# ruihuang1124/CAFE-MPC

Hardware: AMD Instinct MI355X
Metric: DDP iterations/sec, Mini-Cheetah WB N=200, batch=4096; 1/2/4/8 GPU (higher is better)
Workload: dtype f64

## Files before the change

### cafe-mpc_amd/csrc/wb_knot.hpp

```cpp
#pragma once
#include "hs_types.hpp"
#include "wb_model.hpp"
#include "hs_mfma.hpp"

namespace hs {

struct WbCore {
    double x[36], xb[36], u[12], acc[18], tau[18], fext[12], cs[18], sn[18];
    double M[18 * 18];
    double h[18], Jall[12 * 18], Jdv[12], fpos[12], fvel[12];
    double JX[432];
    double gam[12];
    double GG[288 + 2 * MAXG];
    HD double* Jc() { return JX; }
    HD double* Xm() { return JX + 216; }
    HD double* G() { return GG; }
    HD double* LG() { return GG + 144; }
    HD double* gval() { return GG + 288; }
    HD double* bar() { return GG + 288 + MAXG; }
    HD double* dacc() { return GG; }
    HD double* dvel() { return GG + 216; }
    double a0[18], rhs[12], lam[12], qdd[18], grf[12], tmp[64], red[64], rdM[18], rdG[12];
    double wq[48];
    double xnext[36];
// ... 160 lines not shown
        wb_pass<double>(c, L.x, L.x + 18, L.acc, L.cs, L.sn, L.fext, sk);
        if (tid < 12) {
            for (int f = 0; f < 4; f++) if (f != leg) {
                for (int r = 0; r < 3; r++) { L.M[(3 * f + r) * 18 + wb_pj(col)] = 0.0; L.Jall[(3 * f + r) * 18 + col] = 0.0; }
            }
        }
    })
    HS_PHASE(NT, if (tid < 19 && (need_cols || tid == 18)) {
        const int t0 = (tid < 6) ? 12 + 4 * tid : (tid < 18) ? tid - 6 : 36, nt = (tid < 6 || tid == 18) ? 4 : 1;
        V3<double> fb = {0.0, 0.0, 0.0}, nb = fb;
        for (int t = 0; t < nt; t++) { const double* p = L.GG + 6 * (t0 + t); fb = fb + V3<double>{p[0], p[1], p[2]}; nb = nb + V3<double>{p[3], p[4], p[5]}; }
        PSink sk{&L, tid, 0};
        const double c3 = L.cs[3], s3 = L.sn[3], c4 = L.cs[4], s4 = L.sn[4], c5 = L.cs[5], s5 = L.sn[5];
        sk.tau(5, nb.x);
        V3<double> f = rot<0, double>(c5, s5, fb), n = rot<0, double>(c5, s5, nb);
        sk.tau(4, n.y);
        f = rot<1, double>(c4, s4, f); n = rot<1, double>(c4, s4, n);
        sk.tau(3, n.z);
        f = rot<2, double>(c3, s3, f);
        sk.tau(0, f.x); sk.tau(1, f.y); sk.tau(2, f.z);
    })
}

struct Feet4 { int f0, f1, f2, f3; HD int operator[](int i) const { return i == 0 ? f0 : i == 1 ? f1 : i == 2 ? f2 : f3; }
    HD int pick(int i) const { return (((f0 & 3) | (f1 & 3) << 2 | (f2 & 3) << 4 | (f3 & 3) << 6) >> (2 * i)) & 3; } };
HD Feet4 feet_of(PhaseC& P) { int f0 = P.feet[0], f1 = P.feet[1], f2 = P.feet[2], f3 = P.feet[3]; HS_PIN_S(f0); HS_PIN_S(f1); HS_PIN_S(f2); HS_PIN_S(f3); return Feet4{f0, f1, f2, f3}; }
template <class T> HD double pick3(const T& w, int a) { const double w0 = w[0], w1 = w[1], w2 = w[2]; return a == 0 ? w0 : a == 1 ? w1 : w2; }

template <int NT>
HD void wb_select(WbCore& L, int nc, const Feet4& feet, int mode, double alpha) {
    HS_PHASE(NT,
        for (int e = tid; e < 216; e += NT) {
            const int a = e / 18, j = e % 18; const bool act = a < 3 * nc;
            L.Jc()[e] = act ? L.Jall[(3 * feet.pick(act ? a / 3 : 0) + a % 3) * 18 + wb_pi(j)] : 0.0;
        }
        for (int e = tid; e < 144; e += NT) L.G()[e] = (e % 13 == 0) ? 1.0 : 0.0;
        if (tid < 12) {
            const bool act = tid < 3 * nc;
            const int f = act ? feet.pick(tid / 3) : 0, r = tid % 3;
            L.gam[tid] = (act && mode == 0) ? (L.Jdv[3 * f + r] + 2.0 * alpha * L.fvel[3 * f + r]) : 0.0;
            L.grf[tid] = 0.0;
        })
}
template <int NM> HD void wb_gram(WbCore& L, int m, int tid, int nt) {
    for (int e = tid; e < NM * NM; e += nt) {
        const int a = e / NM, b = e % NM;
        double s = 0;
        _Pragma("unroll")
        for (int i = 0; i < 18; i++) s += L.Xm()[i * 12 + a] * L.Xm()[i * 12 + b];
        if (a < m && b < m) L.G()[a * 12 + b] = s;
    }
}

template <int NT, int NM>
HD void wb_kkt_tail(WbCore& L, int m, const Feet4& feet, int mode) {
    HS_PHASE(NT, wb_gram<NM>(L, m, tid, NT);
        if (tid >= 48 && tid < 60) {
            const int a = tid - 48; double s = 0;
            if (mode == 0) { _Pragma("unroll") for (int i = 0; i < 18; i++) s += L.Xm()[i * 12 + a] * L.a0[i]; }
            else { _Pragma("unroll") for (int i = 0; i < 18; i++) s += L.Jc()[a * 18 + i] * L.x[18 + wb_pi(i)]; }
            L.rhs[a] = (a < m) ? (-s - L.gam[a]) : 0.0;
        })
    LQ_STAMP(9)
    chol_f<NT, NM, 12>(L.G(), L.LG(), L.rdG, (mode == 0) ? 1e-12 : 0.0);
    LQ_STAMP(10)
#ifdef HS_HOST_EMU
    HS_PHASE(NT, if (tid == 0) {
        double lam[12];
        _Pragma("unroll")
        for (int i = 0; i < 12; i++) lam[i] = L.rhs[i];
        fwd_s<NM, 12>(L.LG(), L.rdG, lam); bwd_s<NM, 12>(L.LG(), L.rdG, lam);
        double z[18];
        _Pragma("unroll")
        for (int i = 0; i < 18; i++) { double s = L.a0[i]; _Pragma("unroll") for (int a = 0; a < NM; a++) s += L.Xm()[i * 12 + a] * lam[a]; z[i] = s; }
        bwd_s<18, 18, WbNZ>(L.M, L.rdM, z);
        _Pragma("unroll")
        for (int i = 0; i < 18; i++) L.qdd[wb_pi(i)] = z[i] + ((mode == 1) ? L.x[18 + wb_pi(i)] : 0.0);
        _Pragma("unroll")
        for (int a = 0; a < 12; a++) { L.lam[a] = lam[a]; if (a < m) L.grf[3 * feet[a / 3] + a % 3] = lam[a]; }
    })
#else
    HS_PHASE(NT, {
        const int i12 = tid < NM ? tid : NM - 1, i18 = tid < 18 ? tid : 17;
        double lgr[NM], lgc[NM], xr[NM], lmc[6], lleg[3];
        _Pragma("unroll") for (int k = 0; k < NM; k++) { lgr[k] = L.LG()[i12 * 12 + k]; lgc[k] = L.LG()[k * 12 + i12]; xr[k] = L.Xm()[i18 * 12 + k]; }
        const int lg = i18 < 12 ? i18 / 3 : 3, jl = i18 - 3 * lg;
        _Pragma("unroll") for (int k = 0; k < 6; k++) lmc[k] = L.M[(12 + k) * 18 + i18];
        _Pragma("unroll") for (int j = 0; j < 3; j++) lleg[j] = L.M[(3 * lg + j) * 18 + i18];
        const double rg = L.rdG[i12], rm = L.rdM[i18];
        double v = L.rhs[i12];
        _Pragma("unroll") for (int k = 0; k < NM; k++) { const double xk = hs_readlane(v * rg, k); v = (tid == k) ? xk : ((tid > k) ? v - lgr[k] * xk : v); }
        _Pragma("unroll") for (int k = NM - 1; k >= 0; k--) { const double xk = hs_readlane(v * rg, k); v = (tid == k) ? xk : ((tid < k) ? v - lgc[k] * xk : v); }
        double z = L.a0[i18];
        _Pragma("unroll") for (int a = 0; a < NM; a++) z += xr[a] * hs_readlane(v, a);
        _Pragma("unroll") for (int k = 17; k >= 12; k--) { const double xk = hs_readlane(z * rm, k); z = (tid == k) ? xk : ((tid < k) ? z - lmc[k - 12] * xk : z); }
        _Pragma("unroll") for (int j = 2; j >= 0; j--) { const double xk = hs_bperm(z * rm, 3 * lg + j); z = (tid < 12 && jl == j) ? xk : ((tid < 12 && jl < j) ? z - lleg[j] * xk : z); }
        if (tid < 18) L.qdd[wb_pi(tid)] = z + ((mode == 1) ? L.x[18 + wb_pi(tid)] : 0.0);
        if (tid < 12) { const double lm = tid < NM ? v : 0.0; L.lam[tid] = lm; if (tid < m) L.grf[3 * feet.pick(tid / 3) + tid % 3] = lm; }
    })
#endif
}

template <int NT>
HD void wb_kkt_direct(WbCore& L, int nc, const Feet4& feet, int mode, double alpha) {
    const int m = 3 * nc;
    wb_select<NT>(L, nc, feet, mode, alpha);
    LQ_STAMP(7)
#ifdef HS_HOST_EMU
    chol_f<NT, 18, 18, WbNZ>(L.M, L.M, L.rdM, 0.0);
#else
    HS_PHASE(NT, chol_wb18(L.M, L.rdM, tid);)
#endif
    LQ_STAMP(8)
    HS_PHASE(NT, if (tid < 13) {
        const bool isx = tid < 12;
        double* w = reinterpret_cast<double*>(&L);
        constexpr int OXM = offsetof(WbCore, JX) / 8 + 216, OA0 = offsetof(WbCore, a0) / 8;
        double x[18];
        _Pragma("unroll")
        for (int i = 0; i < 18; i++) {
            const double jc = L.Jc()[(isx ? tid : 0) * 18 + i], yv = (mode == 0) ? (L.tau[wb_pi(i)] - L.h[wb_pi(i)]) : 0.0;
            x[i] = isx ? jc : yv;
        }
        fwd_s<18, 18, WbNZ>(L.M, L.rdM, x);
        const int o0 = isx ? OXM + tid : OA0, st = isx ? 12 : 1;
        _Pragma("unroll")
        for (int i = 0; i < 18; i++) w[o0 + i * st] = x[i];
    })
    if (m <= 6) wb_kkt_tail<NT, 6>(L, m, feet, mode); else wb_kkt_tail<NT, 12>(L, m, feet, mode);
}

template <int NM> HD void wb_kkt_column_mid(const WbCore& L, const WbDeriv& D, double* top, double* bot) {
    _Pragma("unroll")
    for (int a = 0; a < NM; a++) {
        double s = -bot[a];
        _Pragma("unroll")
        for (int i = 0; i < 18; i++) s += L.JX[216 + i * 12 + a] * top[i];
        bot[a] = s;
    }
    fwd_s<NM, 12>(D.LGs, D.rdGs, bot); bwd_s<NM, 12>(D.LGs, D.rdGs, bot);
    _Pragma("unroll")
    for (int i = 0; i < 18; i++) {
        double s = top[i];
        _Pragma("unroll")
        for (int a = 0; a < NM; a++) s -= L.JX[216 + i * 12 + a] * bot[a];
        top[i] = s;
    }
}
HD void wb_kkt_column(const WbCore& L, const WbDeriv& D, double* top, double* bot, bool top_is_y, int m) {
    if (!top_is_y) fwd_s<18, 18, WbNZ>(L.M, L.rdM, top);
    if (m <= 6) wb_kkt_column_mid<6>(L, D, top, bot); else wb_kkt_column_mid<12>(L, D, top, bot);
    bwd_s<18, 18, WbNZ>(L.M, L.rdM, top);
}
template <int NT> HD void wb_keep_schur(WbCore& L, WbDeriv& D) {
    chol_f<NT, 12, 12>(L.G(), D.LGs, D.rdGs, 0.0);
}

template <int NT>
HD void wb_dpass(WbCore& L, WbDeriv& D, const ModelDev& md, double grav, double vscale_dyn, double vscale_kin, double ascale_kin, bool q_only, bool chol_g = false) {
    auto base_seed = [](int bs) { return bs < 3 ? 3 + bs : bs < 6 ? 36 + bs : 12 + bs; };
    auto zero_rest = [&](int seed, int leg) {
        for (int f = 0; f < 4; f++) if (f != leg) for (int r = 0; r < 3; r++) {
            D.W[(6 + 3 * f + r) * WT + seed] = 0.0;
            if (seed >= 36) { L.dacc()[(3 * f + r) * 18 + seed - 36] = 0.0; L.dvel()[(3 * f + r) * 18 + seed - 36] = 0.0; }
        }
    };
    HS_PHASE(NT,
        WB_W1_STAMP_BEGIN()
        if (tid < 60 && !(q_only && ((tid >= 12 && tid < 36) || tid >= 48))) {
            const int t = tid; int seed, leg, slot = 0; bool part = t < 36;
            if (t < 12) { seed = base_seed(t >> 2); leg = t & 3; slot = t; }
            else if (t < 36) { const int bs = 6 + ((t - 12) >> 2); seed = base_seed(bs); leg = t & 3; slot = 4 * bs + leg; }
            else { const int jl = (t - 36) % 12; seed = (t < 48 ? 6 : 24) + jl; leg = jl / 3; }
            LaneCfg c = lane_cfg(md, false, 1.0, grav, 0.0, vscale_dyn, 1.0, -1, seed < 18 ? seed : -1, seed >= 18 ? seed - 18 : -1);
            c.l0 = leg; c.l1 = leg + 1; c.body = part && leg == 0; c.partial = part;
            DSink sk{&D, &L, seed, slot};
            wb_pass<Dual, DSink, 1>(c, L.x, L.x + 18, L.acc, L.cs, L.sn, L.fext, sk);
            if (!part) zero_rest(seed, leg);
        }
        const int kt = (NT >= 128) ? tid - 64 : tid;
        if (kt >= 0 && kt < 24) {
            const int t = kt; int seed, leg, slot = 0; const bool part = t < 12;
            if (part) { const int bs = 3 + (t >> 2); seed = base_seed(bs); leg = t & 3; slot = 4 * bs + leg; }
            else { const int jl = t - 12; seed = 42 + jl; leg = jl / 3; }
            LaneCfg c = lane_cfg(md, true, 0.0, 0.0, 1.0, vscale_kin, ascale_kin, -1, seed - 36, -1);
            c.l0 = leg; c.l1 = leg + 1; c.body = false; c.partial = part;
            DSink sk{&D, &L, seed, slot};
            wb_pass<Dual, DSink, 2>(c, L.x, L.x + 18, L.acc, L.cs, L.sn, L.fext, sk);
            if (!part) zero_rest(seed, leg);
        }
        for (int e = tid; e < 108; e += NT) { const int sd = e / 18, i = e % 18; D.W[i * WT + (sd < 3 ? sd : 33 + sd)] = 0.0; }
        for (int e = tid; e < 36; e += NT) { const int j = e / 12, r = e % 12; L.dacc()[r * 18 + j] = 0.0; L.dvel()[r * 18 + j] = 0.0; }
        if (NT >= 128 && chol_g && tid >= 64) WB_CHOL_G(D.LGs, D.rdGs, tid - 64);
        WB_W1_STAMP_END(6))
    HS_PHASE(NT, if (tid < (q_only ? 6 : 12)) {
        const int seed = base_seed(tid), tq = seed < 18 ? seed : seed >= 36 ? seed - 36 : -1;
        V3<Dual> fb = {Dual(0.0), Dual(0.0), Dual(0.0)}, nb = fb;
        for (int l = 0; l < 4; l++) {
            const double* p = D.JPW + 12 * (4 * tid + l);
            fb = fb + V3<Dual>{Dual(p[0], p[1]), Dual(p[2], p[3]), Dual(p[4], p[5])}; nb = nb + V3<Dual>{Dual(p[6], p[7]), Dual(p[8], p[9]), Dual(p[10], p[11])};
        }
        auto SC = [&](int i, Dual& s_, Dual& c_) { const double c0 = L.cs[i], s0 = L.sn[i]; const bool sd = (tq == i); s_ = Dual(s0, sd ? c0 : 0.0); c_ = Dual(c0, sd ? -s0 : 0.0); };
        Dual c3, s3, c4, s4, c5, s5;
        SC(3, s3, c3); SC(4, s4, c4); SC(5, s5, c5);
        DSink sk{&D, &L, seed, 0};
        sk.tau(5, nb.x);
        V3<Dual> f = rot<0>(c5, s5, fb), n = rot<0>(c5, s5, nb);
        sk.tau(4, n.y);
        f = rot<1>(c4, s4, f); n = rot<1>(c4, s4, n);
        sk.tau(3, n.z);
        f = rot<2>(c3, s3, f);
        sk.tau(0, f.x); sk.tau(1, f.y); sk.tau(2, f.z);
    })
}

HD double reb_barrier(double g, double delta) {
    if (g > delta) return -log(g);
    double t = (g - 2 * delta) / delta;
    return .5 * (t * t - 1) - log(delta);
}

HD double wb_constraint(PhaseC& P, const WbCore& L, int c) {
    if (P.go_torque >= 0 && c >= P.go_torque && c < P.go_torque + 24) { int i = c - P.go_torque; return i < 12 ? -L.u[i] + P.torque_limit : L.u[i - 12] + P.torque_limit; }
    if (P.go_jspeed >= 0 && c >= P.go_jspeed && c < P.go_jspeed + 24) { int i = c - P.go_jspeed; return i < 12 ? L.x[24 + i] - P.jspeed_lb : -L.x[24 + i - 12] + P.jspeed_ub; }
    if (P.go_joint >= 0 && c >= P.go_joint && c < P.go_joint + 24) { int i = c - P.go_joint; return i < 12 ? L.x[6 + i] - pick3(P.joint_lb, i % 3) : -L.x[6 + i - 12] + pick3(P.joint_ub, i % 3); }
    if (P.go_height >= 0 && c == P.go_height) return L.x[2] - P.h_min;
    int i = c - P.go_grf, a = i / 5, r = i % 5, f = feet_of(P)[a];
    double fx = L.grf[3 * f], fy = L.grf[3 * f + 1], fz = L.grf[3 * f + 2];
    if (r == 0) return fz;
    if (r == 1) return -fx + P.mu * fz;
    if (r == 2) return fx + P.mu * fz;
    if (r == 3) return -fy + P.mu * fz;
    return fy + P.mu * fz;
}

HD double wb_constraint_sel(PhaseC& P, const WbCore& L, int c) {
    const double* w = reinterpret_cast<const double*>(&L);
    constexpr int OX = offsetof(WbCore, x) / 8, OU = offsetof(WbCore, u) / 8, OG = offsetof(WbCore, grf) / 8;
    const int it = c - P.go_torque, is = c - P.go_jspeed, ij = c - P.go_joint;
    const bool bt = P.go_torque >= 0 && it >= 0 && it < 24, bs = P.go_jspeed >= 0 && is >= 0 && is < 24, bj = P.go_joint >= 0 && ij >= 0 && ij < 24;
    const bool bh = P.go_height >= 0 && c == P.go_height, lin = bt || bs || bj || bh;
    const int i = bt ? it : bs ? is : ij, lo = i < 12 ? i : i - 12;
    const bool up = i >= 12;
    const int a3 = lo % 3;
    const double cj = up ? pick3(P.joint_ub, a3) : -pick3(P.joint_lb, a3);
    const double c0 = bt ? P.torque_limit : bs ? (up ? P.jspeed_ub : -P.jspeed_lb) : bj ? cj : -P.h_min;
    const double sg = bt ? (up ? 1.0 : -1.0) : (bh || !up) ? 1.0 : -1.0;
    const int i1l = bt ? OU + lo : bs ? OX + 24 + lo : bj ? OX + 6 + lo : OX + 2;
    const int ig = lin ? 0 : c - P.go_grf, ga = ig / 5, gr = ig - 5 * ga, f = feet_of(P).pick(ga & 3);
    const int i1 = lin ? i1l : OG + 3 * f + 2, i2 = lin ? i1l : OG + 3 * f + (gr >= 3 ? 1 : 0);
    const double v1 = w[i1], v2 = w[i2];
    const double a = lin ? sg : (gr == 0 ? 1.0 : P.mu);
    const double t2 = lin ? c0 : (gr == 0 ? 0.0 : ((gr == 1 || gr == 3) ? -v2 : v2));
    return hs_fma(a, v1, t2);
}
HD double reb_barrier1(double g, double delta) {
    const bool above = g > delta;
    const double lg = log(above ? g : delta);
    double q = 0.0;
    if (!above) { const double t = (g - 2 * delta) / delta; q = .5 * (t * t - 1); }
    return above ? -lg : q - lg;
}

struct SlotOut { double* cost; double* dsq; double* ming; double* maxh; };

template <int NT, int CNT, int ROWS, class DST, class F>
HD void store_image(DST dst, int tid, F f) {
    constexpr int R = (CNT + NT - 1) / NT;
    const int c0 = tid / ROWS, r0 = tid - ROWS * c0;
    double v[R];
    _Pragma("unroll")
    for (int q = 0; q < R; q++) {
        const int e = tid + NT * q; int r = r0 + (NT * q) % ROWS, c = c0 + (NT * q) / ROWS;
        if (r >= ROWS) { r -= ROWS; c++; }
        v[q] = 0.0;
        if (R * NT == CNT || e < CNT) v[q] = f(e, r, c);
    }
    _Pragma("unroll")
    for (int q = 0; q < R; q++) { const int e = tid + NT * q; if (R * NT == CNT || e < CNT) dst[e] = v[q]; }
}

template <int NT>
HD void wb_rollout_knot(WbCore& L, PhaseC& P, const ModelDev& md, int b, int k, double eps, int reb_active,
                        const double* x0, SlotOut so, size_t slot, int* fail_flag, bool ss = false, bool wr = true) {
    const int h = P.h;
    const size_t kx = ((size_t)b * (h + 1) + k) * 36, ku = ((size_t)b * h + k) * 12;
    double* Kst = L.Jc();
    RL_STAMP0()
    const size_t kk = (size_t)b * h + k;
    struct Late { double kr[7]; } late[HS_NLANES(NT)];
    HS_PHASE(NT,
        const int g = tid < 36 ? 0 : tid < 48 ? 1 : tid < 60 ? 2 : 3, i = tid < 36 ? tid : tid < 48 ? tid - 36 : tid < 60 ? tid - 48 : 0;
        const double* pa = g == 0 ? P.Xbar + kx + i : (g == 1 && !ss) ? P.KdX + ku + i : P.Xbar + kx; const double* pb = P.dX + kx + (g == 0 ? i : 0);
        const double* rr = P.rref + ref_row(P, b, k) * 80;
        const double* pc = rr + tid;
        const double* pd = g == 0 ? P.Xbar + kx + (ss ? 0 : 36) + i : g == 1 ? P.Ubar + ku + i : rr + 64 + i;
        const double* pe = g == 0 ? P.dX + kx + (ss ? 0 : 36) + i : g == 1 ? P.dU + ku + i : rr;
        double va = *pa, vb = *pb, vc = *pc, vd = *pd, ve = *pe;
        const double* pw = tid < 36 ? &P.q[tid] : &P.r[tid < 48 ? tid - 36 : 0];
        const double vw = *pw;
        double er[2], dr[2];
        _Pragma("unroll") for (int q = 0; q < 2; q++) { const int c = q * NT + tid; er[q] = (c < P.ng) ? P.eps[kk * P.ng + c] : 0.0; dr[q] = (c < P.ng) ? P.delta[kk * P.ng + c] : 0.0; }
        if (ss) { Late& lt = late[HS_LANE(tid)]; _Pragma("unroll") for (int q = 0; q < 7; q++) { const int e = q * NT + tid; lt.kr[q] = (e < 432) ? P.K[kk * 432 + e] : 0.0; } }
        HS_CBAR();
        if (tid < 36) {
            const double xb = va, x = ss ? L.xnext[tid] : xb + eps * vb;
// ... 203 lines not shown
    double g = 0;
    for (int f = 0; f < 4; f++) {
        const double* wp = D.wp + 3 * f; const double* wv = D.wv + 3 * f;
        const double* J0 = Jall + (3 * f) * 18; const double* J1 = J0 + 18; const double* J2 = J1 + 18;
        if (wp[0] != 0.0 || wp[1] != 0.0 || wp[2] != 0.0) {
            const bool in = d >= 3 && d < 18; const int dd = in ? d : 3;
            const double t0 = in ? wp[0] * J0[dd] : 0.0, t1 = in ? wp[1] * J1[dd] : 0.0, t2 = in ? wp[2] * J2[dd] : 0.0;
            g += t0 * D.ep[3 * f] + t1 * D.ep[3 * f + 1] + t2 * D.ep[3 * f + 2];
            _Pragma("unroll")
            for (int i = 3; i < 18; i++) acc[i] += J0[i] * t0 + J1[i] * t1 + J2[i] * t2;
        }
        if (wv[0] != 0.0 || wv[1] != 0.0 || wv[2] != 0.0) {
            const double* V0 = dvel + (3 * f) * 18; const double* V1 = V0 + 18; const double* V2 = V1 + 18;
            const int dd = d < 18 ? d : d - 18;
            const double t0 = wv[0] * (d < 18 ? V0[dd] : J0[dd]), t1 = wv[1] * (d < 18 ? V1[dd] : J1[dd]), t2 = wv[2] * (d < 18 ? V2[dd] : J2[dd]);
            g += t0 * D.ev[3 * f] + t1 * D.ev[3 * f + 1] + t2 * D.ev[3 * f + 2];
            _Pragma("unroll")
            for (int i = 0; i < 18; i++) { acc[i] += V0[i] * t0 + V1[i] * t1 + V2[i] * t2; acc[18 + i] += J0[i] * t0 + J1[i] * t1 + J2[i] * t2; }
        }
    }
    _Pragma("unroll")
    for (int i = 0; i < 36; i++) colout[i * 36] = acc[i];
    return g;
}

#ifndef HS_HOST_EMU
HD void wb_cost_gram_acc(WbCore& L, WbDeriv& D, int lane, d4_t (&c)[3][3]) {
    const int li = lane & 15, lk = lane >> 4;
    bool anyv = false;
    _Pragma("unroll") for (int a = 0; a < 12; a++) anyv = anyv || (D.wv[a] != 0.0);
    _Pragma("unroll") for (int ti = 0; ti < 3; ti++) _Pragma("unroll") for (int tj = 0; tj < 3; tj++) c[ti][tj] = d4_t{0.0, 0.0, 0.0, 0.0};
    _Pragma("unroll") for (int kg = 0; kg < 6; kg++) {
        if (kg >= 3 && !anyv) break;
        const int k = 4 * kg + lk, r = (kg < 3) ? k : k - 12;
        const double w = (kg < 3) ? D.wp[r] : D.wv[r], res = (kg < 3) ? D.ep[r] : D.ev[r];
        double e[3];
        _Pragma("unroll") for (int t = 0; t < 3; t++) {
            const int col = 16 * t + li, cc = col < 36 ? col : 35, lo = cc < 18, c18 = lo ? cc : cc - 18;
            const double vj = L.Jall[r * 18 + c18];
            if (kg < 3) e[t] = (cc >= 3 && lo && col < 36) ? vj : 0.0;
            else { const double vd = L.dvel()[r * 18 + c18]; e[t] = col < 36 ? (lo ? vd : vj) : 0.0; }
        }
        _Pragma("unroll") for (int ti = 0; ti < 3; ti++) {
            const double a = w * e[ti];
            _Pragma("unroll") for (int tj = 0; tj < 3; tj++) {
                const double bb = (tj == 2 && li == 4) ? res : e[tj];
                c[ti][tj] = __builtin_amdgcn_mfma_f64_16x16x4f64(a, bb, c[ti][tj], 0, 0, 0);
            }
        }
    }
}
#endif
template <int NT>
HD void wb_cost_gram(WbLqLds& S, double* gvec) {
    WbCore& L = S.c; WbDeriv& D = S.d;
#ifdef HS_HOST_EMU
    HS_PHASE_L(NT, if (tid < 37) {
        const int j = tid;
        auto E = [&](int k, int c) { if (k < 12) return (c >= 3 && c < 18) ? L.Jall[k * 18 + c] : 0.0; const int r = k - 12; return c < 18 ? L.dvel()[r * 18 + c] : L.Jall[r * 18 + c - 18]; };
        for (int i = 0; i < 36; i++) {
            double s = 0;
            for (int k = 0; k < 24; k++) { const double w = k < 12 ? D.wp[k] : D.wv[k - 12]; s += w * E(k, i) * (j < 36 ? E(k, j) : (k < 12 ? D.ep[k] : D.ev[k - 12])); }
            if (j < 36) D.W[i * 36 + j] = s; else gvec[i] = s;
        }
    })
#else
    HS_PHASE_L(NT, if (tid < 64) {
        const int li = tid & 15, lk = tid >> 4;
        d4_t c[3][3];
        wb_cost_gram_acc(L, D, tid, c);
        _Pragma("unroll") for (int ti = 0; ti < 3; ti++) _Pragma("unroll") for (int tj = 0; tj < 3; tj++) _Pragma("unroll") for (int q = 0; q < 4; q++) {
            const int row = 16 * ti + lk + 4 * q, col = 16 * tj + li;
            if (row < 36) { if (col < 36) D.W[row * 36 + col] = c[ti][tj][q]; else if (col == 36) gvec[row] = c[ti][tj][q]; }
        }
    })
#endif
}

#define KC_REGION(s_, e_, ptr_) if (NT * q + NT - 1 >= (s_) && NT * q < (e_)) { if (NT * q >= (s_) && NT * q + NT - 1 < (e_)) (ptr_)[i - (s_)] = v; else if (i >= (s_) && i < (e_)) (ptr_)[i - (s_)] = v; }
template <int NT>
HD void wb_lq_knot(WbLqLds& S, PhaseC& P, const ModelDev& md, int b, int k, int reb_active, bool cached = false) {
    WbCore& L = S.c; WbDeriv& D = S.d;
    const int h = P.h; const double dt = P.dt;
    const size_t kx = ((size_t)b * (h + 1) + k) * 36, ku = ((size_t)b * h + k) * 12, kk = (size_t)b * h + k, rw = ref_row(P, b, k);
    LQ_STAMP0()
    HS_PHASE(NT,
        const double vx = (tid < 36) ? P.X[kx + tid] : 0.0, vu = (tid < 12) ? P.U[ku + tid] : 0.0;
        const double vt = (tid < 36) ? P.xr[rw * 36 + tid] : (tid < 48) ? P.ur[rw * 12 + tid - 36] : 0.0;
        const double vf = (tid < 12) ? P.foot_pos[rw * 12 + tid] : (tid < 15) ? P.body_pos[rw * 3 + tid - 12] : (tid < 19) ? (double)P.ref_contact[rw * 4 + tid - 15] : 0.0;
        const double vv = (tid < 12) ? P.foot_vel[rw * 12 + tid] : 0.0;
        const double vw = (tid < 36) ? P.q[tid] : (tid < 48) ? P.r[tid - 36] : 0.0;
        double gr[2], dr[2], er[2];
        _Pragma("unroll") for (int q = 0; q < 2; q++) { const int c = q * NT + tid; const size_t gi = kk * P.ng + c; const bool in = c < P.ng; gr[q] = in ? P.g[gi] : 1.0; dr[q] = in ? P.delta[gi] : 1.0; er[q] = in ? P.eps[gi] : 0.0; }
        double r[KC_SIZE / NT];
        if (cached) {
            const double* kc = P.kc + kk * KC_SIZE;
            _Pragma("unroll") for (int q = 0; q < KC_SIZE / NT; q++) r[q] = kc[q * NT + tid];
        }
        HS_CBAR();
        if (tid < 36) L.x[tid] = vx; if (tid < 12) { L.u[tid] = vu; L.fext[tid] = 0.0; }
        if (tid < 18) { L.acc[tid] = 0.0; L.tau[tid] = 0.0; }
        if (tid < 48) { L.tmp[tid] = vt; L.wq[tid] = vw; }
        if (tid < 12) { L.red[tid] = vf; L.red[12 + tid] = vv; } else if (tid < 15) L.red[12 + tid] = vf; else if (tid < 19) L.red[13 + tid] = vf;
        _Pragma("unroll") for (int q = 0; q < 2; q++) {
            const int c = q * NT + tid; const double g = gr[q], delta = dr[q], e = er[q]; double bd, bdd;
            if (g > delta) { bd = -1.0 / g; bdd = 1.0 / (g * g); } else { bd = (g - 2 * delta) / delta / delta; bdd = 1.0 / (delta * delta); }
            if (c < P.ng) { D.bd()[c] = reb_active ? e * bd : 0.0; D.bdd()[c] = reb_active ? e * bdd : 0.0; }
        }
        if (cached) {
            if (tid < 18) { double sv, cv; sincos_(vx, sv, cv); L.cs[tid] = cv; L.sn[tid] = sv; }
            _Pragma("unroll") for (int q = 0; q < KC_SIZE / NT; q++) {
                const int i = q * NT + tid; const double v = r[q];
                KC_REGION(KC_M, KC_X, L.M) KC_REGION(KC_X, KC_LG, L.Xm()) KC_REGION(KC_LG, KC_RDM, D.LGs) KC_REGION(KC_RDM, KC_RDG, L.rdM)
                KC_REGION(KC_QDD, KC_GRF, L.qdd) KC_REGION(KC_GRF, KC_LAM, L.grf) KC_REGION(KC_LAM, KC_J, L.lam)
                KC_REGION(KC_J, KC_FP, L.Jall) KC_REGION(KC_FP, KC_FV, L.fpos) KC_REGION(KC_FV, KC_FV + 12, L.fvel)
            }
        })
    LQ_STAMP(11)
    if (cached) {
        if (NT < 128) chol_f<NT, 12, 12>(D.LGs, D.LGs, D.rdGs, 0.0);
        LQ_STAMP(0)
    } else {
        HS_PHASE(NT, if (tid < 12) L.tau[6 + tid] = L.u[tid];)
        wb_terms<NT>(L, md, true);
        LQ_STAMP(0)
        wb_kkt_direct<NT>(L, P.nc, feet_of(P), 0, P.bg_alpha);
        wb_keep_schur<NT>(L, D);
    }
    LQ_STAMP(1)
    const int m = 3 * P.nc;
    HS_PHASE(NT, if (tid < 18) L.acc[tid] = L.qdd[tid]; if (tid < 12) L.fext[tid] = L.grf[tid];)
    wb_dpass<NT>(L, D, md, GRAV, 1.0, 1.0, 1.0, false, cached);
    LQ_STAMP(2)
    if (NT >= 128) {
        HS_WPHASE_W(0, if (tid < 48) {
        const int d = tid;
        double top[18], bot[12];
        {
            const int dc = d < 36 ? d : 35, c = dc < 18 ? dc : dc - 18, d2 = d < 18 ? d : 0;
            double w1[18], w2[18], vg[12], vd[12], vj[12];
            _Pragma("unroll") for (int i = 0; i < 18; i++) { w1[i] = D.W[wb_pi(i) * WT + dc]; w2[i] = D.W[wb_pi(i) * WT + 36 + d2]; }
            const Feet4 ft = feet_of(P);
            _Pragma("unroll") for (int a = 0; a < 12; a++) {
                const int r = 3 * ft[a / 3] + a % 3;
                vg[a] = L.G()[r * 18 + c]; vd[a] = L.dvel()[r * 18 + c]; vj[a] = L.Jall[r * 18 + c];
            }
            HS_CBAR();
            _Pragma("unroll") for (int i = 0; i < 18; i++) top[i] = (d < 36) ? (w1[i] + ((d < 18) ? w2[i] : 0.0)) : ((wb_pi(i) == 6 + d - 36) ? 1.0 : 0.0);
            _Pragma("unroll") for (int a = 0; a < 12; a++) {
                const double t1 = dc < 18 ? vg[a] : 2.0 * vd[a], t2 = dc < 18 ? vd[a] : vj[a];
                bot[a] = (a < m && d < 36) ? t1 + 2.0 * P.bg_alpha * t2 : 0.0;
            }
        }
        wb_kkt_column(L, D, top, bot, false, m);
        if (d < 36) {
            _Pragma("unroll")
            for (int i = 0; i < 18; i++) D.W[WR0 + wb_pi(i) * 36 + d] = -top[i] * dt + ((d == 18 + wb_pi(i)) ? 1.0 : 0.0);
            _Pragma("unroll")
            for (int a = 0; a < 12; a++) D.stC()[a + 12 * d] = 0.0;
            for (int a = 0; a < m; a++) D.stC()[(3 * P.feet[a / 3] + a % 3) + 12 * d] = bot[a];
        } else {
            const int j = d - 36;
            _Pragma("unroll")
            for (int i = 0; i < 18; i++) D.stB()[wb_pi(i) + 18 * j] = top[i] * dt;
            _Pragma("unroll")
            for (int a = 0; a < 12; a++) D.stD()[a + 12 * j] = 0.0;
            for (int a = 0; a < m; a++) D.stD()[(3 * P.feet[a / 3] + a % 3) + 12 * j] = -bot[a];
        }
        })
        LQ_STAMP(3)
        double* const T1 = L.Jc();
        WB_W1_STAMP_BEGIN()
        HS_WPHASE_W(1, wb_cost_blocks_lane(S, P, false, tid);
            if (tid < 36) {
                const int d = tid;
                double lxd = dt * L.wq[d] * (L.x[d] - L.tmp[d]);
                double diag = dt * L.wq[d];
                if (P.go_joint >= 0 && d >= 6 && d < 18) {
                    const int i = d - 6;
                    lxd += dt * (D.bd()[P.go_joint + i] - D.bd()[P.go_joint + 12 + i]); diag += dt * (D.bdd()[P.go_joint + i] + D.bdd()[P.go_joint + 12 + i]);
                }
                if (P.go_height >= 0 && d == 2) { lxd += dt * D.bd()[P.go_height]; diag += dt * D.bdd()[P.go_height]; }
                if (P.go_jspeed >= 0 && d >= 24) {
                    const int i = d - 24;
                    lxd += dt * (D.bd()[P.go_jspeed + i] - D.bd()[P.go_jspeed + 12 + i]); diag += dt * (D.bdd()[P.go_jspeed + i] + D.bdd()[P.go_jspeed + 12 + i]);
                }
                T1[d] = lxd; T1[36 + d] = diag;
            })
#ifdef HS_HOST_EMU
        static double emu_tile[1296];
        HS_WPHASE_W(1, if (tid < 37) {
            const int j = tid;
            auto E = [&](int k2, int c) { if (k2 < 12) return (c >= 3 && c < 18) ? L.Jall[k2 * 18 + c] : 0.0; const int r = k2 - 12; return c < 18 ? L.dvel()[r * 18 + c] : L.Jall[r * 18 + c - 18]; };
            for (int i = 0; i < 36; i++) {
                double sm = 0;
                for (int k2 = 0; k2 < 24; k2++) { const double w = k2 < 12 ? D.wp[k2] : D.wv[k2 - 12]; sm += w * E(k2, i) * (j < 36 ? E(k2, j) : (k2 < 12 ? D.ep[k2] : D.ev[k2 - 12])); }
                if (j < 36) emu_tile[i * 36 + j] = sm; else T1[120 + i] = sm;
            }
        })
        HS_WPHASE_W(1, if (tid < 36) { emu_tile[tid * 36 + tid] += T1[36 + tid]; P.lx[kk * P.rs + tid] = T1[tid] + T1[120 + tid]; })
        HS_WPHASE_W(1, store_image<64, 1296, 36>(P.lxx + kk * P.rs, tid, [&](int, int r, int c) { return emu_tile[c * 36 + r]; });)
#else
        HS_WPHASE_W(1, {
            const int li = tid & 15, lk = tid >> 4;
            d4_t c[3][3];
            wb_cost_gram_acc(L, D, tid, c);
            _Pragma("unroll") for (int ti = 0; ti < 3; ti++) _Pragma("unroll") for (int tj = 0; tj < 3; tj++) _Pragma("unroll") for (int q = 0; q < 4; q++) {
                const int row = 16 * ti + lk + 4 * q, col = 16 * tj + li;
                if (row < 36) {
                    if (col < 36) { double v = c[ti][tj][q]; if (row == col) v += T1[36 + row]; P.lxx[kk * P.rs + col + 36 * row] = v; }
                    else if (col == 36) P.lx[kk * P.rs + row] = T1[row] + c[ti][tj][q];
                }
            }
        })
#endif
        HS_WPHASE_W(1, if (tid < 12) {
            const int i = tid;
            double lu = dt * L.wq[36 + i] * (L.u[i] - L.tmp[36 + i]), luu = dt * L.wq[36 + i];
            if (P.go_torque >= 0) { lu += dt * (-D.bd()[P.go_torque + i] + D.bd()[P.go_torque + 12 + i]); luu += dt * (D.bdd()[P.go_torque + i] + D.bdd()[P.go_torque + 12 + i]); }
            P.lu[kk * P.rs + i] = lu; T1[72 + i] = luu;
            double ly = 0.0, b0 = 0.0, b1 = 0.0, b2 = 0.0; const int f = i / 3, r = i % 3; int a = -1; for (int t = 0; t < P.nc; t++) if (P.feet[t] == f) a = t;
            if (P.go_grf >= 0 && a >= 0) {
                const double mu = P.mu;
                for (int c = 0; c < 5; c++) {
                    const double r0 = (c == 1) ? -1.0 : (c == 2) ? 1.0 : 0.0, r1 = (c == 3) ? -1.0 : (c == 4) ? 1.0 : 0.0, r2 = (c == 0) ? 1.0 : mu;
                    const double rr = (r == 0) ? r0 : (r == 1) ? r1 : r2;
                    const double hb = dt * D.bdd()[P.go_grf + 5 * a + c] * rr;
                    ly += D.bd()[P.go_grf + 5 * a + c] * rr;
                    b0 += hb * r0; b1 += hb * r1; b2 += hb * r2;
                }
            }
            T1[84 + 3 * i] = b0; T1[85 + 3 * i] = b1; T1[86 + 3 * i] = b2;
            P.ly[kk * P.rs + i] = dt * ly;
        })
        HS_WPHASE_W(1, store_image<64, 144, 12>(P.luu + kk * P.rs, tid, [&](int, int r, int c) { return r == c ? T1[72 + r] : 0.0; });
                       store_image<64, 144, 12>(P.lyy + kk * P.rs, tid, [&](int, int r, int c) { return (r / 3 == c / 3) ? T1[84 + (r % 3) + 3 * c] : 0.0; });)
        WB_W1_STAMP_END(5)
        hs_phase_sync_all<NT>();
        HS_PHASE_L(NT,
            store_image<NT, 648, 18>(P.A + kk * P.rs, tid, [&](int, int r, int c) { return D.W[WR0 + r * 36 + c]; });
            store_image<NT, 432, 36>(P.C + kk * P.rs, tid, [&](int e, int, int) { return D.stC()[e]; });
            store_image<NT, 216, 18>(P.B + kk * P.rs, tid, [&](int e, int, int) { return D.stB()[e]; });
            store_image<NT, 144, 12>(P.D + kk * P.rs, tid, [&](int e, int, int) { return D.stD()[e]; });)
        LQ_STAMP(4)
        return;
    }
    HS_PHASE(NT, if (tid < 48) {
        const int d = tid;
        double top[18], bot[12];
        {
            const int dc = d < 36 ? d : 35, c = dc < 18 ? dc : dc - 18, d2 = d < 18 ? d : 0;
            double w1[18], w2[18], vg[12], vd[12], vj[12];
            _Pragma("unroll") for (int i = 0; i < 18; i++) { w1[i] = D.W[wb_pi(i) * WT + dc]; w2[i] = D.W[wb_pi(i) * WT + 36 + d2]; }
            const Feet4 ft = feet_of(P);
            _Pragma("unroll") for (int a = 0; a < 12; a++) {
                const int r = 3 * ft[a / 3] + a % 3;
                vg[a] = L.G()[r * 18 + c]; vd[a] = L.dvel()[r * 18 + c]; vj[a] = L.Jall[r * 18 + c];
            }
            HS_CBAR();
            _Pragma("unroll") for (int i = 0; i < 18; i++) top[i] = (d < 36) ? (w1[i] + ((d < 18) ? w2[i] : 0.0)) : ((wb_pi(i) == 6 + d - 36) ? 1.0 : 0.0);
            _Pragma("unroll") for (int a = 0; a < 12; a++) {
                const double t1 = dc < 18 ? vg[a] : 2.0 * vd[a], t2 = dc < 18 ? vd[a] : vj[a];
                bot[a] = (a < m && d < 36) ? t1 + 2.0 * P.bg_alpha * t2 : 0.0;
            }
        }
        wb_kkt_column(L, D, top, bot, false, m);
        if (d < 36) {
            _Pragma("unroll")
            for (int i = 0; i < 18; i++) D.W[WR0 + wb_pi(i) * 36 + d] = -top[i] * dt + ((d == 18 + wb_pi(i)) ? 1.0 : 0.0);
            _Pragma("unroll")
            for (int a = 0; a < 12; a++) D.stC()[a + 12 * d] = 0.0;
            for (int a = 0; a < m; a++) D.stC()[(3 * P.feet[a / 3] + a % 3) + 12 * d] = bot[a];
        } else {
            const int j = d - 36;
            _Pragma("unroll")
            for (int i = 0; i < 18; i++) D.stB()[wb_pi(i) + 18 * j] = top[i] * dt;
            _Pragma("unroll")
            for (int a = 0; a < 12; a++) D.stD()[a + 12 * j] = 0.0;
            for (int a = 0; a < m; a++) D.stD()[(3 * P.feet[a / 3] + a % 3) + 12 * j] = -bot[a];
        }
    })
    LQ_STAMP(3)
    HS_PHASE_L(NT,
        store_image<NT, 648, 18>(P.A + kk * P.rs, tid, [&](int, int r, int c) { return D.W[WR0 + r * 36 + c]; });
        store_image<NT, 432, 36>(P.C + kk * P.rs, tid, [&](int e, int, int) { return D.stC()[e]; });
        store_image<NT, 216, 18>(P.B + kk * P.rs, tid, [&](int e, int, int) { return D.stB()[e]; });
        store_image<NT, 144, 12>(P.D + kk * P.rs, tid, [&](int e, int, int) { return D.stD()[e]; });)
    LQ_STAMP(4)
    wb_cost_blocks<NT>(S, P, k, false);
    wb_cost_gram<NT>(S, D.JPW);
    HS_PHASE_L(NT, if (tid < 36) {
        const int d = tid;
        double lxd = dt * L.wq[d] * (L.x[d] - L.tmp[d]);
        double diag = dt * L.wq[d];
        lxd += D.JPW[d];
        if (P.go_joint >= 0 && d >= 6 && d < 18) {
            const int i = d - 6;
            lxd += dt * (D.bd()[P.go_joint + i] - D.bd()[P.go_joint + 12 + i]); diag += dt * (D.bdd()[P.go_joint + i] + D.bdd()[P.go_joint + 12 + i]);
        }
        if (P.go_height >= 0 && d == 2) { lxd += dt * D.bd()[P.go_height]; diag += dt * D.bdd()[P.go_height]; }
        if (P.go_jspeed >= 0 && d >= 24) {
            const int i = d - 24;
            lxd += dt * (D.bd()[P.go_jspeed + i] - D.bd()[P.go_jspeed + 12 + i]); diag += dt * (D.bdd()[P.go_jspeed + i] + D.bdd()[P.go_jspeed + 12 + i]);
        }
        D.W[d * 36 + d] += diag;
        P.lx[kk * P.rs + d] = lxd;
    })
    HS_PHASE_L(NT, store_image<NT, 1296, 36>(P.lxx + kk * P.rs, tid, [&](int, int r, int c) { return D.W[r * 36 + c]; });)
    LQ_STAMP(5)
    HS_PHASE_L(NT, for (int i = tid; i < 288; i += NT) L.Jc()[i] = 0.0;)
    HS_PHASE_L(NT, if (tid < 12) {
        const int i = tid;
        double lu = dt * L.wq[36 + i] * (L.u[i] - L.tmp[36 + i]), luu = dt * L.wq[36 + i];
        if (P.go_torque >= 0) { lu += dt * (-D.bd()[P.go_torque + i] + D.bd()[P.go_torque + 12 + i]); luu += dt * (D.bdd()[P.go_torque + i] + D.bdd()[P.go_torque + 12 + i]); }
        P.lu[kk * P.rs + i] = lu; L.Jc()[i + 12 * i] = luu;
        double ly = 0.0; const int f = i / 3, r = i % 3; int a = -1; for (int t = 0; t < P.nc; t++) if (P.feet[t] == f) a = t;
        if (P.go_grf >= 0 && a >= 0) {
            const double mu = P.mu;
            for (int c = 0; c < 5; c++) {
                const double r0 = (c == 1) ? -1.0 : (c == 2) ? 1.0 : 0.0, r1 = (c == 3) ? -1.0 : (c == 4) ? 1.0 : 0.0, r2 = (c == 0) ? 1.0 : mu;
                const double rr = (r == 0) ? r0 : (r == 1) ? r1 : r2;
                const double hb = dt * D.bdd()[P.go_grf + 5 * a + c] * rr;
                ly += D.bd()[P.go_grf + 5 * a + c] * rr;
                L.Jc()[144 + (3 * f) + 12 * i] += hb * r0; L.Jc()[144 + (3 * f + 1) + 12 * i] += hb * r1; L.Jc()[144 + (3 * f + 2) + 12 * i] += hb * r2;
            }
        }
        P.ly[kk * P.rs + i] = dt * ly;
    })
    HS_PHASE_L(NT, store_image<NT, 144, 12>(P.luu + kk * P.rs, tid, [&](int e, int, int) { return L.Jc()[e]; });
                   store_image<NT, 144, 12>(P.lyy + kk * P.rs, tid, [&](int e, int, int) { return L.Jc()[144 + e]; });)
    LQ_STAMP(6)
}

template <int NT>
HD void wb_lq_terminal(WbLqLds& S, PhaseC& P, PhaseC* Pn, const ModelDev& md, int b, int al_active) {
    WbCore& L = S.c; WbDeriv& D = S.d;
    const int h = P.h;
    const size_t kx = ((size_t)b * (h + 1) + h) * 36;
    HS_PHASE(NT, if (tid < 36) L.x[tid] = P.X[kx + tid]; if (tid < 18) { L.acc[tid] = 0.0; L.tau[tid] = 0.0; } if (tid < 12) L.fext[tid] = 0.0;
             wb_cost_prefetch(L, P, b, h, tid);)
    wb_terms<NT>(L, md, true);
    wb_dpass<NT>(L, D, md, 0.0, 1.0, 1.0, 0.0, true);
    wb_cost_blocks<NT>(S, P, h, true);
    HS_PHASE(NT, if (tid < 36) {
        const int d = tid;
        double px = P.qf[d] * (L.x[d] - L.tmp[d]);
        px += wb_cost_column(D, L.Jall, L.dvel(), d, D.W + d);
        double diag = P.qf[d];
        if (al_active && P.nt > 0) {
            int t = 0;
            for (int f = 0; f < 4; f++) if (P.td[f]) {
                const double sg = P.sigma[(size_t)b * P.nt + t], lm = P.lambda[(size_t)b * P.nt + t], hh = P.th[(size_t)b * P.nt + t];
                const double hd = d < 18 ? L.Jall[(3 * f + 2) * 18 + d] : 0.0;
                px += (sg * hh + lm) * hd;
                for (int i = 0; i < 18; i++) D.W[i * 36 + d] += (sg * (1 + hh) + lm) * (L.Jall[(3 * f + 2) * 18 + i] * hd);
                t++;
            }
        }
        D.W[d * 36 + d] += diag;
        P.Phix[(size_t)b * 36 + d] = px;
    })
    HS_PHASE(NT, for (int e = tid; e < 1296; e += NT) { const int r = e % 36, c = e / 36; P.Phixx[(size_t)b * 1296 + e] = D.W[r * 36 + c]; })
    if (Pn == nullptr) return;
    const int nn = Pn->n;
    if (!P.has_impact) {
        HS_PHASE(NT, for (int i = tid; i < nn * 36; i += NT) { int r = i % nn, c = i / nn; int src = (nn == 36) ? r : (r < 6 ? r : r + 12); P.Px[(size_t)b * nn * 36 + i] = (src == c) ? 1.0 : 0.0; })
        return;
    }
    int tdfeet[4] = {0, 0, 0, 0}; int ntd = 0; for (int f = 0; f < 4; f++) if (P.td[f]) tdfeet[ntd++] = f;
    const int m = 3 * ntd;
    wb_kkt_direct<NT>(L, ntd, Feet4{tdfeet[0], tdfeet[1], tdfeet[2], tdfeet[3]}, 1, 0.0);
    wb_keep_schur<NT>(L, D);
    HS_PHASE(NT, if (tid < 18) L.acc[tid] = L.qdd[tid] - L.x[18 + tid]; if (tid < 12) L.fext[tid] = 0.0;)
    HS_PHASE(NT, if (tid == 0) { double pad[16]; for (int i = 0; i < 16; i++) pad[i] = i < m ? L.lam[i] : 0.0;
                 for (int i = 0; i < ntd; i++) for (int d = 0; d < 3; d++) L.fext[3 * tdfeet[i] + d] = pad[i + d]; })
    wb_dpass<NT>(L, D, md, 0.0, 0.0, 0.0, 0.0, true);
    HS_PHASE(NT, if (tid < 18) for (int i = 0; i < 18; i++) D.W[i * WT + tid] += D.W[i * WT + 36 + tid];)
    HS_PHASE(NT, if (tid < 18) { L.xb[tid] = L.x[18 + tid]; })
    HS_PHASE(NT, if (tid < 18) { L.x[18 + tid] = L.qdd[tid]; })
    HS_PHASE(NT, if (tid >= 36 && tid < 54) {
        LaneCfg c = lane_cfg(md, true, 0.0, 0.0, 0.0, 1.0, 0.0, -1, tid - 36, -1);
        struct VSink { WbCore* C; int j; HD void tau(int, const Dual&) const {} HD void base(const V3<Dual>&, const V3<Dual>&) const {} HD void foot(int f, const V3<Dual>&, const V3<Dual>& v, const V3<Dual>&) const {
            C->dvel()[(3 * f) * 18 + j] = v.x.d; C->dvel()[(3 * f + 1) * 18 + j] = v.y.d; C->dvel()[(3 * f + 2) * 18 + j] = v.z.d; } } sk{&L, tid - 36};
        wb_pass<Dual>(c, L.x, L.x + 18, L.acc, L.cs, L.sn, L.fext, sk);
    })
    HS_PHASE(NT, if (tid < 36) {
        const int d = tid;
        double top[18], bot[12];
        _Pragma("unroll")
        for (int i = 0; i < 18; i++) {
            if (d < 18) top[i] = D.W[wb_pi(i) * WT + d];
            else { const int j = wb_pj(d - 18); top[i] = (i < j) ? L.M[j * 18 + i] : (i == j) ? 1.0 / L.rdM[j] : 0.0; }
        }
        _Pragma("unroll")
        for (int a = 0; a < 12; a++) bot[a] = (d < 18 && a < m) ? L.dvel()[(3 * tdfeet[a / 3] + a % 3) * 18 + d] : 0.0;
        wb_kkt_column(L, D, top, bot, d >= 18, m);
        _Pragma("unroll")
        for (int i = 0; i < 18; i++) D.W[WR0 + wb_pi(i) * 36 + d] = (d < 18) ? -top[i] : top[i];
    })
    HS_PHASE(NT, for (int e = tid; e < nn * 36; e += NT) {
        const int r = e % nn, c = e / nn;
        double v;
        if (nn == 36) v = (r < 18) ? ((r == c) ? 1.0 : 0.0) : D.W[WR0 + (r - 18) * 36 + c];
        else v = (r < 6) ? ((r == c) ? 1.0 : 0.0) : D.W[WR0 + (r - 6) * 36 + c];
        P.Px[(size_t)b * nn * 36 + e] = v;
    })
}

}
```

Before: 98790.

## Software-pipeline KKT column solve with double-buffered register staging of shared operands

Replaces the monolithic KKT column solve (forward/back substitution with M, Jacobian products, Schur-complement triangular solves) with a compile-time chunked plan. Each chunk's shared-memory operands are loaded into a register double buffer while the previous chunk computes, so LDS latency overlaps with FMA work. The change raises register pressure through two 24-double buffers per thread, which may reduce occupancy or cause spills in f64. It is enabled by default through LQ_COL_STAGE.

```diff
diff --git a/cafe-mpc_amd/csrc/wb_knot.hpp b/cafe-mpc_amd/csrc/wb_knot.hpp
--- a/cafe-mpc_amd/csrc/wb_knot.hpp
+++ b/cafe-mpc_amd/csrc/wb_knot.hpp
@@ -336,6 +336,114 @@
     if (m <= 6) wb_kkt_column_mid<6>(L, D, top, bot); else wb_kkt_column_mid<12>(L, D, top, bot);
     bwd_s<18, 18, WbNZ>(L.M, L.rdM, top);
 }
+#ifndef LQ_COL_STAGE
+#define LQ_COL_STAGE 1
+#endif
+#ifndef LQ_COL_BUF
+#define LQ_COL_BUF 24
+#endif
+constexpr int COL_BUF = LQ_COL_BUF, COL_FB = COL_BUF >= 36 ? 2 : 1, COL_XR = COL_BUF >= 36 ? 18 : 9;
+enum { COL_FWD18, COL_XTY, COL_FWDG, COL_BWDG, COL_YXN, COL_BWD18 };
+struct ColChunk { int piece, r0, r1, h0, h1; };
+template <int NM> HD constexpr int col_gsplit(int j) { return j == 0 ? 0 : NM == 6 ? 6 : COL_BUF >= 36 ? (j == 1 ? 7 : j == 2 ? 10 : 12) : 4 + 2 * j; }
+template <int NM> struct ColPlan {
+    static constexpr int NF = 1 + 6 / COL_FB, XH = 18 / COL_XR, NX = NM / 2 * XH, NG = NM == 6 ? 1 : COL_BUF >= 36 ? 3 : 4, RY = NM == 12 ? COL_BUF / 12 : COL_BUF >= 36 ? 6 : 3, NY = 18 / RY;
+    static constexpr int N = NF + NX + 2 * NG + NY + 5;
+    static constexpr ColChunk chunk(int c) {
+        if (c < NF) return ColChunk{COL_FWD18, c == 0 ? 0 : 12 + COL_FB * (c - 1), 12 + COL_FB * c, 0, 0};
+        c -= NF; if (c < NX) return ColChunk{COL_XTY, 2 * (c / XH), 2 * (c / XH) + 2, COL_XR * (c % XH), COL_XR * (c % XH) + COL_XR};
+        c -= NX; if (c < NG) return ColChunk{COL_FWDG, col_gsplit<NM>(c), col_gsplit<NM>(c + 1), 0, 0};
+        c -= NG; if (c < NG) return ColChunk{COL_BWDG, col_gsplit<NM>(c), col_gsplit<NM>(c + 1), 0, 0};
+        c -= NG; if (c < NY) return ColChunk{COL_YXN, RY * c, RY * c + RY, 0, 0};
+        c -= NY; return ColChunk{COL_BWD18, c == 0 ? 0 : 3 + 3 * c, 6 + 3 * c, 0, 0};
+    }
+};
+template <int NM, int C> HD void col_load(const WbCore& L, const WbDeriv& D, double* buf) {
+    constexpr ColChunk ch = ColPlan<NM>::chunk(C);
+    int n = 0;
+    if (ch.piece == COL_FWD18) {
+        _Pragma("unroll") for (int i = ch.r0; i < ch.r1; i++) { _Pragma("unroll") for (int k = 0; k < i; k++) if (WbNZ::nz(i, k)) buf[n++] = L.M[i * 18 + k]; buf[n++] = L.rdM[i]; }
+    } else if (ch.piece == COL_XTY) {
+        _Pragma("unroll") for (int i = ch.h0; i < ch.h1; i++) { _Pragma("unroll") for (int a = ch.r0; a < ch.r1; a++) buf[n++] = L.JX[216 + i * 12 + a]; }
+    } else if (ch.piece == COL_FWDG) {
+        _Pragma("unroll") for (int i = ch.r0; i < ch.r1; i++) { _Pragma("unroll") for (int k = 0; k < i; k++) buf[n++] = D.LGs[i * 12 + k]; buf[n++] = D.rdGs[i]; }
+    } else if (ch.piece == COL_BWDG) {
+        _Pragma("unroll") for (int t = ch.r0; t < ch.r1; t++) { const int i = NM - 1 - t; _Pragma("unroll") for (int k = i + 1; k < NM; k++) buf[n++] = D.LGs[k * 12 + i]; buf[n++] = D.rdGs[i]; }
+    } else if (ch.piece == COL_YXN) {
+        _Pragma("unroll") for (int i = ch.r0; i < ch.r1; i++) { _Pragma("unroll") for (int a = 0; a < NM; a++) buf[n++] = L.JX[216 + i * 12 + a]; }
+    } else {
+        _Pragma("unroll") for (int t = ch.r0; t < ch.r1; t++) { const int i = 17 - t; _Pragma("unroll") for (int k = i + 1; k < 18; k++) if (WbNZ::nz(k, i)) buf[n++] = L.M[k * 18 + i]; buf[n++] = L.rdM[i]; }
+    }
+}
+template <int NM, int C> HD void col_compute(const double* buf, double* top, double* bot) {
+    constexpr ColChunk ch = ColPlan<NM>::chunk(C);
+    int n = 0;
+    if (ch.piece == COL_FWD18) {
+        _Pragma("unroll") for (int i = ch.r0; i < ch.r1; i++) {
+            double s = top[i];
+            _Pragma("unroll") for (int k = 0; k < i; k++) if (WbNZ::nz(i, k)) s -= buf[n++] * top[k];
+            top[i] = s * buf[n++];
+        }
+        HS_PIN(top[ch.r1 - 1]);
+    } else if (ch.piece == COL_XTY) {
+        _Pragma("unroll") for (int a = ch.r0; a < ch.r1; a++) {
+            double s = ch.h0 == 0 ? -bot[a] : bot[a];
+            _Pragma("unroll") for (int i = ch.h0; i < ch.h1; i++) s += buf[(i - ch.h0) * (ch.r1 - ch.r0) + a - ch.r0] * top[i];
+            bot[a] = s; HS_PIN(bot[a]);
+        }
+    } else if (ch.piece == COL_FWDG) {
+        _Pragma("unroll") for (int i = ch.r0; i < ch.r1; i++) {
+            double s = bot[i];
+            _Pragma("unroll") for (int k = 0; k < i; k++) s -= buf[n++] * bot[k];
+            bot[i] = s * buf[n++];
+        }
+        HS_PIN(bot[ch.r1 - 1]);
+    } else if (ch.piece == COL_BWDG) {
+        _Pragma("unroll") for (int t = ch.r0; t < ch.r1; t++) {
+            const int i = NM - 1 - t; double s = bot[i];
+            _Pragma("unroll") for (int k = i + 1; k < NM; k++) s -= buf[n++] * bot[k];
+            bot[i] = s * buf[n++];
+        }
+        HS_PIN(bot[NM - ch.r1]);
+    } else if (ch.piece == COL_YXN) {
+        _Pragma("unroll") for (int i = ch.r0; i < ch.r1; i++) {
+            double s = top[i];
+            _Pragma("unroll") for (int a = 0; a < NM; a++) s -= buf[n++] * bot[a];
+            top[i] = s; HS_PIN(top[i]);
+        }
+    } else {
+        _Pragma("unroll") for (int t = ch.r0; t < ch.r1; t++) {
+            const int i = 17 - t; double s = top[i];
+            _Pragma("unroll") for (int k = i + 1; k < 18; k++) if (WbNZ::nz(k, i)) s -= buf[n++] * top[k];
+            top[i] = s * buf[n++];
+        }
+        HS_PIN(top[18 - ch.r1]);
+    }
+}
+template <int NM, int C, int CE> HD void col_run(const WbCore& L, const WbDeriv& D, double* top, double* bot, double (&buf)[2][COL_BUF]) {
+    if constexpr (C < CE) {
+        if constexpr (C + 1 < CE) col_load<NM, C + 1>(L, D, buf[(C + 1) & 1]);
+        HS_CBAR();
+        col_compute<NM, C>(buf[C & 1], top, bot);
+        col_run<NM, C + 1, CE>(L, D, top, bot, buf);
+    }
+}
+template <int NM, bool Y_LANES> HD void col_solve(const WbCore& L, const WbDeriv& D, double* top, double* bot, bool top_is_y) {
+    constexpr int NF = ColPlan<NM>::NF, N = ColPlan<NM>::N;
+    double buf[2][COL_BUF];
+    if (Y_LANES) {
+        if (!top_is_y) { col_load<NM, 0>(L, D, buf[0]); col_run<NM, 0, NF>(L, D, top, bot, buf); }
+        col_load<NM, NF>(L, D, buf[NF & 1]); col_run<NM, NF, N>(L, D, top, bot, buf);
+    } else { col_load<NM, 0>(L, D, buf[0]); col_run<NM, 0, N>(L, D, top, bot, buf); }
+}
+template <bool Y_LANES = false>
+HD void wb_kkt_column_st(const WbCore& L, const WbDeriv& D, double* top, double* bot, bool top_is_y, int m) {
+#if LQ_COL_STAGE
+    if (m <= 6) col_solve<6, Y_LANES>(L, D, top, bot, top_is_y); else col_solve<12, Y_LANES>(L, D, top, bot, top_is_y);
+#else
+    wb_kkt_column(L, D, top, bot, top_is_y, m);
+#endif
+}
 template <int NT> HD void wb_keep_schur(WbCore& L, WbDeriv& D) {
     chol_f<NT, 12, 12>(L.G(), D.LGs, D.rdGs, 0.0);
 }
@@ -845,7 +953,7 @@
                 bot[a] = (a < m && d < 36) ? t1 + 2.0 * P.bg_alpha * t2 : 0.0;
             }
         }
-        wb_kkt_column(L, D, top, bot, false, m);
+        wb_kkt_column_st(L, D, top, bot, false, m);
         if (d < 36) {
             _Pragma("unroll")
             for (int i = 0; i < 18; i++) D.W[WR0 + wb_pi(i) * 36 + d] = -top[i] * dt + ((d == 18 + wb_pi(i)) ? 1.0 : 0.0);
@@ -957,7 +1065,7 @@
                 bot[a] = (a < m && d < 36) ? t1 + 2.0 * P.bg_alpha * t2 : 0.0;
             }
         }
-        wb_kkt_column(L, D, top, bot, false, m);
+        wb_kkt_column_st(L, D, top, bot, false, m);
         if (d < 36) {
             _Pragma("unroll")
             for (int i = 0; i < 18; i++) D.W[WR0 + wb_pi(i) * 36 + d] = -top[i] * dt + ((d == 18 + wb_pi(i)) ? 1.0 : 0.0);
@@ -1087,7 +1195,7 @@
         }
         _Pragma("unroll")
         for (int a = 0; a < 12; a++) bot[a] = (d < 18 && a < m) ? L.dvel()[(3 * tdfeet[a / 3] + a % 3) * 18 + d] : 0.0;
-        wb_kkt_column(L, D, top, bot, d >= 18, m);
+        wb_kkt_column_st<true>(L, D, top, bot, d >= 18, m);
         _Pragma("unroll")
         for (int i = 0; i < 18; i++) D.W[WR0 + wb_pi(i) * 36 + d] = (d < 18) ? -top[i] : top[i];
     })
```

New measurement: 99520, median of 6. Within noise of the previous version (+0.7%).
